# OpenGene/repaq

Hardware: AMD Instinct MI355X
Metric: raw FASTQ MB/s encode+decode (higher is better)
Workload: dtype u8; 1 GPU; configs[2]: synthetic NovaSeq PE150 two files (-i/-I), 2 x 4.01 GB FASTQ (fqgen profile 1, 11200000 pairs, seed 3, N 20 ppm), -k 1000, encode + decode; chunks_per_gpu=3360, parity=unchecked (checked with --full)

## Files before the change

repaq_amd/csrc/enc/chunk_flags_overlap.h:

```cpp
#pragma once
struct Layout {
    uint32_t off_readlens, off_n1lens, off_n2lens, off_stlens, off_lanes, off_tiles, off_x, off_y, off_n1, off_n2, off_st, off_seq, off_qual, off_ov, off_npos;
    uint32_t total, msize, seq_size, qual_size, npos_size, n1_size, n2_size, st_size, x_size, y_size, n_reads, flags;
};
__device__ __forceinline__ uint32_t name2_len_of(const Text& T, const ReadTab& R, uint32_t g) { return line_len(T, g, 0) - R.name2_off[g]; }

#define CF_ALL 0x3FFu
__global__ void k_chunk_flags_a(Text T, ReadTab R, ChunkTab C, const DevHeader* __restrict__ D, int is_pe, uint32_t* __restrict__ cbits, uint32_t* __restrict__ cfail) {
    __shared__ uint8_t s_names[4 * 65 * NAME_STRIDE];
    const uint32_t c = blockIdx.y, f = C.first[c], e = C.first[c + 1];
    const int l = lane_id(), w = wave_id(); const uint32_t wpb = blockDim.x >> 6;
    uint8_t* rows = s_names + (size_t)w * 65 * NAME_STRIDE;
    const bool can0 = is_pe && D->support_interleaved; const uint32_t dpos = D->name2_diff_pos, dch = D->name2_diff_char;
    const uint32_t nl0 = line_len(T, f, 0); const uint8_t* nm0g = line_ptr(T, f, 0);
    const uint32_t n1l0 = R.name1_len[f], n2o0 = R.name2_off[f], n2l0 = nl0 - n2o0, len0 = R.len[f], stl0 = line_len(T, f, 2);
    const uint8_t* st0 = line_ptr(T, f, 2); const uint8_t lane0 = R.lane[f]; const uint16_t tile0 = R.tile[f];
    { const uint32_t take = nl0 < NAME_CAP ? nl0 : NAME_CAP; for (uint32_t i = (uint32_t)l; i < take; i += 64) rows[64 * NAME_STRIDE + i] = nm0g[i]; }
    const uint8_t* nm0 = nl0 <= NAME_CAP ? rows + 64 * NAME_STRIDE : nm0g;
    uint32_t bits = CF_ALL, fail = 0xFFFFFFFFu;
    for (uint32_t gb = f + (blockIdx.x * wpb + (uint32_t)w) * 64u; gb < e; gb += gridDim.x * wpb * 64u) {
        const uint32_t g = gb + (uint32_t)l; const bool v = g < e;
        uint32_t nb = 0, nl = 0, stb = 0, stl = 0; int s = 0;
        if (v) { uint32_t r; read_loc(T, g, s, r); const uint32_t* p = t_lo(T, s) + 4 * (size_t)r; nb = p[0]; nl = p[1] - 1 - nb; stb = p[2]; stl = p[3] - 1 - stb; }
        wave_lds_sync();
// ... 314 lines not shown
__global__ void __launch_bounds__(256) k_chunk_prefix(Text T, ReadTab R, ChunkTab C, const DevHeader* __restrict__ D, const int16_t* __restrict__ ovraw,
        int8_t* __restrict__ ovb) {
    const uint32_t c = blockIdx.x, f = C.first[c], e = C.first[c + 1], tid = threadIdx.x;
    const bool enc = C.il[c] != 0 && (D->flags & H_PE_OVERLAP); const int shift = D->overlap_shift;
    const uint32_t fl = C.flags[c];
    const bool pieces = !(fl & C_NAME1_SAME) || ((D->flags & H_NAME2) && !(fl & C_NAME2_SAME)) || !(fl & C_STRAND_SAME);
    U4 carry; carry.a = carry.b = carry.c = carry.d = 0;
    for (uint32_t base = f; base < e; base += 1024u) {
        U4 v[4]; U4 acc; acc.a = acc.b = acc.c = acc.d = 0;
#pragma unroll
        for (int i = 0; i < 4; i++) {
            const uint32_t g = base + 4u * tid + (uint32_t)i; v[i].a = v[i].b = v[i].c = v[i].d = 0;
            if (g < e) {
                uint32_t st = R.len[g];
                if (enc && ((g - f) & 1u)) {
                    int ov = ovraw[g >> 1];
                    if (ov + shift > 127) ov = 0;
                    if (ov + shift < -127) ov = 0;
                    ovb[g >> 1] = (int8_t)(ov + shift); st -= (uint32_t)(ov < 0 ? -ov : ov); R.stored[g] = st;
                }
                if (pieces) { int s_; uint32_t r_; read_loc(T, g, s_, r_); const uint4 lo4 = *(const uint4*)(t_lo(T, s_) + 4 * (size_t)r_);
                        v[i].a = R.name1_len[g]; v[i].b = (lo4.y - 1u - lo4.x) - R.name2_off[g]; v[i].c = lo4.w - 1u - lo4.z; }
                v[i].d = st;
                acc = acc + v[i];
            }
        }
        U4 tot; U4 run = carry + block_excl_sum<U4>(acc, &tot);
#pragma unroll
        for (int i = 0; i < 4; i++) { const uint32_t g = base + 4u * tid + (uint32_t)i; if (g < e) { if (pieces) R.pv[g] = run; R.sd[g] = run.d; run = run + v[i]; } }
        carry = carry + tot;
    }
    if (tid == 0) { C.ptot[c] = carry; C.sbase[c] = C.qbase[c]; }
}
__global__ void k_chunk_ptot(ReadTab R, ChunkTab C, uint32_t n_chunks) {
    const uint32_t c = blockIdx.x * blockDim.x + threadIdx.x;
    if (c < n_chunks) C.ptot[c] = R.pv[C.first[c + 1]] - R.pv[C.first[c]];
}
```

repaq_amd/csrc/enc/gather_tiles.h:

```cpp
#pragma once
#define G2_CAP 23552u
#define G2_SE_OK 1
#define G2_CNT 256u
struct __attribute__((packed, aligned(1))) GU16g { uint32_t a, b, c, d; };
__device__ __forceinline__ void pack4_codes(uint32_t w, uint32_t& code, uint32_t& nb, uint32_t& bad) {
    const uint32_t idx = (w >> 1) & 0x03030303u;
    const uint32_t ok = eq_bytes_full(__builtin_amdgcn_perm(0u, 0x47544341u, idx), w);
    code = ((__builtin_amdgcn_perm(0u, 0x00020301u, idx) & ok) * 0x01041040u) >> 24;
    nb = 0; bad = 0;
    if (ok != 0xFFFFFFFFu) { const uint32_t isn = eq_bytes_full(w, 0x4E4E4E4Eu); nb = ((isn & 0x01010101u) * 0x01020408u) >> 24;
            bad = (((~ok & ~isn) & 0x01010101u) * 0x01020408u) >> 24; }
}
__device__ __forceinline__ void pack4_codes_rc(uint32_t w, uint32_t& code, uint32_t& nb) {
    const uint32_t u = w & 0xDFDFDFDFu, idx = (u >> 1) & 0x03030303u;
    const uint32_t ok = eq_bytes_full(__builtin_amdgcn_perm(0u, 0x47544341u, idx), u);
    code = ((__builtin_amdgcn_perm(0u, 0x03010002u, idx) & ok) * 0x01041040u) >> 24;
    nb = ((~ok & 0x01010101u) * 0x01020408u) >> 24;
}
__device__ __forceinline__ bool pack16_fast(const uint32_t (&w)[4], uint32_t& code) {
    uint32_t diff = 0; code = 0;
#pragma unroll
    for (int i = 0; i < 4; i++) {
        const uint32_t idx = (w[i] >> 1) & 0x03030303u;
        diff |= __builtin_amdgcn_perm(0u, 0x47544341u, idx) ^ w[i];
// ... 433 lines not shown
    const uint32_t nw = (pq[first[c + 1]] - pq[first[c]] + 31u) >> 5; const size_t w0 = (size_t)(qbase[c] >> 5);
    for (uint32_t v = 0; v < G2_PLANES; v++) if (!((dense_mask >> v) & 1u)) for (uint32_t i = threadIdx.x; i < nw; i += blockDim.x) planes[(size_t)v * pstride + w0 + i] = 0u;
}
__global__ void k_gather_redo_reset(const uint32_t* __restrict__ only, uint32_t* __restrict__ segm, int* __restrict__ segc, uint32_t n_seg,
                                    uint32_t* __restrict__ xplane, uint64_t pstride, const DevHeader* __restrict__ D, uint32_t nd, const uint32_t* __restrict__ pq, const uint32_t* __restrict__ first, const uint64_t* __restrict__ qbase) {
    const uint32_t c = blockIdx.x; if (!only[c]) return;
    const size_t k = (size_t)c * MAX_STREAMS * n_seg;
    for (uint32_t i = threadIdx.x; i < MAX_STREAMS * n_seg; i += blockDim.x) { segm[k + i] = 0u; segc[k + i] = -1; }
    if (xplane) { k_rare_zero_chunk(xplane, pstride, dense_mask_of(D, nd), pq, first, qbase, c);
            if (threadIdx.x == 0) xplane[(size_t)G2_PLANES * pstride + (size_t)c * (1u + G2_RARE_LIST)] = 0u; }
}
__global__ void k_rare_cleanup(uint32_t* __restrict__ rare, uint32_t* __restrict__ planes, uint64_t pstride, const DevHeader* __restrict__ D, uint32_t nd,
        const uint32_t* __restrict__ pq, const uint32_t* __restrict__ first, const uint64_t* __restrict__ qbase) {
    const uint32_t c = blockIdx.x; uint32_t* const rc = rare + (size_t)c * (1u + G2_RARE_LIST); const uint32_t n = rc[0]; if (!n) return;
    if (n <= G2_RARE_LIST) { const size_t w0 = (size_t)(qbase[c] >> 5); for (uint32_t i = threadIdx.x; i < n; i += blockDim.x) { const uint32_t e = rc[1u + i];
            planes[(size_t)(e >> 28) * pstride + w0 + (e & 0x0FFFFFFFu)] = 0u; } }
    else k_rare_zero_chunk(planes, pstride, dense_mask_of(D, nd), pq, first, qbase, c);
    __syncthreads();
    if (threadIdx.x == 0) rc[0] = 0u;
}
__device__ __forceinline__ uint32_t loose_codes(const uint32_t* __restrict__ lpk, uint32_t ld, uint32_t b) {
    const uint32_t d = ld + (b >> 4), sh = 2u * (b & 15u); const uint32_t lo = lpk[d];
    return sh ? (uint32_t)(((((unsigned long long)lpk[d + 1]) << 32) | lo) >> sh) : lo;
}
__device__ __forceinline__ uint32_t loose_nbits(const uint16_t* __restrict__ lnb, uint32_t ld, uint32_t b) {
    const uint32_t d = ld + (b >> 4), sh = b & 15u; const uint32_t lo = lnb[d];
    return (sh ? ((((uint32_t)lnb[d + 1]) << 16) | lo) >> sh : lo) & 0xFFFFu;
}
#define SP_OWN 4096u
#define SP_EXTRA 8u
#define SP_U 3
struct __attribute__((packed, aligned(4))) SpU8 { uint32_t a, b; };
struct __attribute__((packed, aligned(2))) SpU4 { uint32_t a; };
__global__ void __launch_bounds__(256) k_seqpack(const uint32_t* __restrict__ pq, const uint32_t* __restrict__ sd, const U4* __restrict__ ptot,
        const uint32_t* __restrict__ first, const uint32_t* __restrict__ ilv, const int8_t* __restrict__ ovb,
                                                 const DevHeader* __restrict__ D, const uint64_t* __restrict__ sbase, const uint32_t* __restrict__ lpk, const uint16_t* __restrict__ lnb, const uint8_t* __restrict__ rn,
                                                 uint32_t* __restrict__ spk, uint16_t* __restrict__ snm, uint32_t* __restrict__ ncount, uint32_t* __restrict__ nmap, uint32_t* __restrict__ segm, int* __restrict__ segc, uint32_t n_seg,
                                                 uint32_t rshift) {
    __shared__ uint32_t s_sd[256 + SP_EXTRA + 1], s_ld[256 + SP_EXTRA], s_sk[256 + SP_EXTRA]; __shared__ uint8_t s_own[SP_OWN];
    __shared__ uint8_t s_hn[256 + SP_EXTRA + 8];
    const uint32_t c = blockIdx.y, f = first[c], e = first[c + 1], tid = threadIdx.x;
    const uint32_t ps0 = sd[f], S = ptot[c].d;
    const bool il = ilv[c] != 0, enc = il && (D->flags & H_PE_OVERLAP); const int shift = D->overlap_shift;
    uint32_t* const ok = spk + (size_t)(sbase[c] >> 4); uint16_t* const on = snm + (size_t)(sbase[c] >> 4);
    const uint32_t nshift = nmap_shift(S); uint32_t* const nm = nmap + (size_t)c * NMAP_WORDS;
    const size_t nsi = ((size_t)c * MAX_STREAMS + NPOS_SLOT) * n_seg;
    uint32_t nsum = 0;
    auto skip_of = [&](uint32_t g) -> uint32_t {
        if (enc && ((g - f) & 1u)) { const int ov = (int)ovb[g >> 1] - shift; if (ov > 0) return (uint32_t)ov; }
        return 0u;
    };
    const uint32_t R = 1u << rshift;
    for (uint32_t r0 = f + blockIdx.x * R; r0 < e; r0 += gridDim.x * R) {
        const uint32_t nr = e - r0 < R ? e - r0 : R, nx = e - r0 < R + SP_EXTRA ? e - r0 : R + SP_EXTRA;
        for (uint32_t t = tid; t <= nx; t += blockDim.x) {
            const uint32_t g = r0 + t; s_sd[t] = g < e ? sd[g] - ps0 : S;
            if (t < nx) { s_ld[t] = (pq[g] >> 4) + g; s_sk[t] = skip_of(g); s_hn[t] = rn[g]; } else s_hn[t] = 0;
        }
        __syncthreads();
        const uint32_t kbase = (s_sd[0] + 15u) >> 4, kend = (s_sd[nr] + 15u) >> 4;
        if (tid < nr) { const uint32_t ka = (s_sd[tid] + 15u) >> 4, kb = (s_sd[tid + 1] + 15u) >> 4; for (uint32_t k = ka; k < kb; k++) s_own[k - kbase] = (uint8_t)tid; }
        __syncthreads();
        const uint32_t ndw = kend - kbase;
        for (uint32_t i0 = 0; i0 < ndw; i0 += blockDim.x * SP_U) {
            struct Dw { uint32_t k, need, t1, jj, sh, sh2, take2, n, n2; unsigned long long c, c2; } q[SP_U]; uint32_t nres[SP_U];
#pragma unroll
            for (int u = 0; u < SP_U; u++) nres[u] = 0;
#pragma unroll
            for (int u = 0; u < SP_U; u++) {
                Dw& x = q[u]; x.need = 0; x.take2 = 0; x.k = x.t1 = x.jj = x.sh = x.sh2 = x.n = x.n2 = 0; x.c = x.c2 = 0;
                const uint32_t i = i0 + (uint32_t)u * blockDim.x + tid;
                if (i < ndw) {
                    const uint32_t k = kbase + i, j = s_own[i];
                    const uint32_t B = 16u * k, si = B - s_sd[j], need = S - B < 16u ? S - B : 16u, av = s_sd[j + 1] - B, t1 = need < av ? need : av;
                    const uint32_t b0 = s_sk[j] + si, d = s_ld[j] + (b0 >> 4);
                    x.k = k; x.need = need; x.t1 = t1; x.sh = b0 & 15u; x.jj = j + 1u;
                    { const SpU8 v = *(const SpU8*)(lpk + d); x.c = (((unsigned long long)v.b) << 32) | v.a; x.n = s_hn[j] ? ((const SpU4*)(lnb + d))->a : 0u; }
                    if (t1 < need && j + 1u < nx) {
                        const uint32_t avail = s_sd[j + 2] - s_sd[j + 1]; x.jj = j + 2u;
                        if (avail) {
                            const uint32_t s2 = s_sk[j + 1], d2 = s_ld[j + 1] + (s2 >> 4); x.sh2 = s2 & 15u; x.take2 = avail < need - t1 ? avail : need - t1;
                            const SpU8 v = *(const SpU8*)(lpk + d2); x.c2 = (((unsigned long long)v.b) << 32) | v.a; x.n2 = s_hn[j + 1] ? ((const SpU4*)(lnb + d2))->a : 0u;
                        }
                    }
                }
            }
#pragma unroll
            for (int u = 0; u < SP_U; u++) {
                const Dw& x = q[u];
                if (!x.need) continue;
                const uint32_t k = x.k, B = 16u * k, need = x.need;
                unsigned long long acc = (uint32_t)(x.c >> (2u * x.sh)) & (x.t1 >= 16u ? 0xFFFFFFFFu : (1u << (2u * x.t1)) - 1u);
                uint32_t nacc = ((x.n >> x.sh) & 0xFFFFu) & ((1u << x.t1) - 1u);
                uint32_t filled = x.t1, jj = x.jj;
                if (x.take2) {
                    acc |= (unsigned long long)((uint32_t)(x.c2 >> (2u * x.sh2)) & (x.take2 >= 16u ? 0xFFFFFFFFu : (1u << (2u * x.take2)) - 1u)) << (2u * filled);
                    nacc |= (((x.n2 >> x.sh2) & 0xFFFFu) & ((1u << x.take2) - 1u)) << filled; filled += x.take2;
                }
                while (filled < need) {
                    uint32_t a, b, l2, s2;
                    if (jj < nx) { a = s_sd[jj]; b = s_sd[jj + 1]; l2 = s_ld[jj]; s2 = s_sk[jj]; }
                    else { const uint32_t gg = r0 + jj; a = sd[gg] - ps0; b = gg + 1u < e ? sd[gg + 1] - ps0 : S; l2 = (pq[gg] >> 4) + gg; s2 = skip_of(gg); }
                    const uint32_t avail = b - a;
                    if (avail) {
                        const uint32_t take = avail < need - filled ? avail : need - filled;
                        acc |= (unsigned long long)(loose_codes(lpk, l2, s2) & (take >= 16u ? 0xFFFFFFFFu : (1u << (2u * take)) - 1u)) << (2u * filled);
                        if (jj < nx ? s_hn[jj] : rn[r0 + jj]) nacc |= (loose_nbits(lnb, l2, s2) & ((1u << take) - 1u)) << filled;
                        filled += take;
                    }
                    jj++;
                }
                ok[k] = (uint32_t)acc; on[k] = (uint16_t)nacc; nres[u] = nacc;
            }
#pragma unroll
            for (int u = 0; u < SP_U; u++) {
                const uint32_t na = q[u].need ? nres[u] : 0u;
                const unsigned long long hn = __ballot(na != 0u);
                if (!hn) continue;
                const uint32_t B = 16u * q[u].k, sg = B / PC_SEG_POS, mb = (B >> 12) >> nshift, n = (uint32_t)__popc(na);
                const int lead = __ffsll((long long)hn) - 1;
                const uint32_t sg0 = (uint32_t)__shfl((int)sg, lead), mb0 = (uint32_t)__shfl((int)mb, lead);
                const bool mine = na != 0u && sg == sg0; const int last = na ? (int)(B + 31u - (uint32_t)__clz((int)na)) : -1;
                const uint32_t sum = wave_sum<uint32_t>(mine ? n : 0u); const int mx = wave_max<int>(mine ? last : -1);
                if (lane_id() == lead) { atomicAdd(&segm[nsi + sg0], sum); atomicMax(&segc[nsi + sg0], mx); atomicOr(&nm[mb0 >> 5], 1u << (mb0 & 31u)); }
                if (na != 0u && !mine) { atomicAdd(&segm[nsi + sg], n); atomicMax(&segc[nsi + sg], last); }
                if (na != 0u && mb != mb0) atomicOr(&nm[mb >> 5], 1u << (mb & 31u));
                nsum += n;
            }
        }
        __syncthreads();
    }
    nsum = wave_sum(nsum);
    if (lane_id() == 0 && nsum) atomicAdd(&ncount[c], nsum);
}
// ... 47 lines not shown
```

repaq_amd/csrc/rfq_api.hip:

```cpp
#include "rfq_ctx.h"
#include <cstring>
#include <algorithm>
#include <new>
#include <cstdlib>
#include <string>
#include <cerrno>

extern "C" const char* rfq_version(void) {
#ifdef RFQ_SIMT_EMULATION
    return "rfq_hip 0.1.0 simt-emulation (test build, not a product path)";
#else
    return "rfq_hip 0.1.0 gfx950";
#endif
}

static bool opt_num(const std::string& v, long long lo, long long hi, long long* out) {
    if (v.empty()) return false;
    errno = 0; char* end = nullptr; const long long x = strtoll(v.c_str(), &end, 10);
    if (errno || !end || *end || end == v.c_str() || x < lo || x > hi) return false;
    *out = x; return true;
}
extern "C" int rfq_set_option(rfq_ctx* c, const char* name, const char* value) {
    if (!c || !name) return RFQ_E_ARG;
    const std::string n = name, v = value ? value : ""; const bool set = !v.empty(); const RfqOpts d; long long num = 0;
#define RFQ_OPT_NUM(LO, HI, WHAT) if (set && !opt_num(v, LO, HI, &num)) return rfq_fail(c, RFQ_E_ARG, "%s is " WHAT " (got \"%s\")", name, v.c_str());
    if (n == "RFQ_GATHER") { if (set && v != "old" && v != "tile") return rfq_fail(c, RFQ_E_ARG, "RFQ_GATHER is old or tile"); c->opt.gather_old = v == "old"; }
    else if (n == "RFQ_QUAL") { if (set && v != "bytes" && v != "masks") return rfq_fail(c, RFQ_E_ARG, "RFQ_QUAL is bytes or masks"); c->opt.qual_bytes = v == "bytes"; }
    else if (n == "RFQ_CODER") { if (set && v != "list" && v != "mask") return rfq_fail(c, RFQ_E_ARG, "RFQ_CODER is list or mask");
            c->opt.coder = v == "list" ? 1 : (v == "mask" ? 2 : 0); }
    else if (n == "RFQ_INDEX") { if (set && v != "2pass" && v != "1pass") return rfq_fail(c, RFQ_E_ARG, "RFQ_INDEX is 2pass or 1pass"); c->opt.index_2pass = v == "2pass"; }
    else if (n == "RFQ_IDX_TILES") { if (set && v != "4" && v != "8" && v != "16") return rfq_fail(c, RFQ_E_ARG, "RFQ_IDX_TILES is 4, 8 or 16");
            c->opt.idx_tiles = set ? atoi(v.c_str()) : d.idx_tiles; }
    else if (n == "RFQ_STREAMS") { if (set && v != "1" && v != "2") return rfq_fail(c, RFQ_E_ARG, "RFQ_STREAMS is 1 or 2"); c->opt.one_stream = v == "1"; }
    else if (n == "RFQ_SLICE_BYTES") { RFQ_OPT_NUM(1024, 0xFFFFFFF0ll - 16, "a number of bytes in 1024 .. 2^32 - 32") c->opt.slice_bytes = set ? (size_t)num : 0; }
    else if (n == "RFQ_SLICE_BASES") { RFQ_OPT_NUM(1, 0xFFFFFFF0ll, "a number of bases in 1 .. 2^32 - 16") c->opt.slice_bases = set ? (uint64_t)num : 0; }
    else if (n == "RFQ_WALK") { if (set && v != "exact" && v != "guess") return rfq_fail(c, RFQ_E_ARG, "RFQ_WALK is guess or exact"); c->opt.walk_exact = v == "exact"; }
    else if (n == "RFQ_GW_SHIFT") { RFQ_OPT_NUM(4, 30, "4 .. 30") c->opt.gw_shift = set ? (int)num : d.gw_shift; }
    else if (n == "RFQ_MATERIALISE") { if (set && v != "0" && v != "1") return rfq_fail(c, RFQ_E_ARG, "RFQ_MATERIALISE is 0 or 1"); c->opt.materialise = v == "1"; }
    else if (n == "RFQ_TRACE") { if (set && v != "0" && v != "1") return rfq_fail(c, RFQ_E_ARG, "RFQ_TRACE is 0 or 1"); c->opt.trace = v == "1"; }
    else if (n == "RFQ_G2_PAD") { RFQ_OPT_NUM(0, 150000, "0 .. 150000 bytes of LDS") c->opt.g2_pad = set ? (uint32_t)num : 0u; }
    else if (n == "RFQ_SP_PAD") { RFQ_OPT_NUM(0, 150000, "0 .. 150000 bytes of LDS") c->opt.sp_pad = set ? (uint32_t)num : d.sp_pad; }
    else if (n == "RFQ_POS_SEG") { if (set && v != "1024" && v != "2048") return rfq_fail(c, RFQ_E_ARG, "RFQ_POS_SEG is 1024 or 2048"); c->opt.pos_seg = set ? atoi(v.c_str()) : 0; }
    else if (n == "RFQ_SPEC") { if (set && v != "0" && v != "1") return rfq_fail(c, RFQ_E_ARG, "RFQ_SPEC is 0 or 1"); c->opt.no_spec = v == "0"; }
    else return rfq_fail(c, RFQ_E_ARG, "unknown option %s", name);
#undef RFQ_OPT_NUM
    return RFQ_OK;
}
static const char* const RFQ_OPTION_NAMES[] = { "RFQ_GATHER", "RFQ_QUAL", "RFQ_CODER", "RFQ_INDEX", "RFQ_IDX_TILES", "RFQ_STREAMS", "RFQ_SLICE_BYTES", "RFQ_SLICE_BASES", "RFQ_WALK", "RFQ_GW_SHIFT", "RFQ_MATERIALISE", "RFQ_TRACE", "RFQ_G2_PAD", "RFQ_SP_PAD", "RFQ_POS_SEG", "RFQ_SPEC" };
extern "C" const char* rfq_option_name(int i) { return (i >= 0 && i < (int)(sizeof RFQ_OPTION_NAMES / sizeof RFQ_OPTION_NAMES[0])) ? RFQ_OPTION_NAMES[i] : nullptr; }
extern "C" int rfq_get_option(const rfq_ctx* c, const char* name, char* out, size_t cap) {
    if (!c || !name || !out || !cap) return RFQ_E_ARG;
    const std::string n = name; const RfqOpts& o = c->opt; const RfqOpts d; std::string v;
    if (n == "RFQ_GATHER") v = o.gather_old ? "old" : "";
    else if (n == "RFQ_QUAL") v = o.qual_bytes ? "bytes" : "";
    else if (n == "RFQ_CODER") v = o.coder == 1 ? "list" : (o.coder == 2 ? "mask" : "");
    else if (n == "RFQ_INDEX") v = o.index_2pass ? "2pass" : "";
    else if (n == "RFQ_IDX_TILES") v = o.idx_tiles != d.idx_tiles ? std::to_string(o.idx_tiles) : "";
    else if (n == "RFQ_STREAMS") v = o.one_stream ? "1" : "";
    else if (n == "RFQ_SLICE_BYTES") v = o.slice_bytes ? std::to_string(o.slice_bytes) : "";
    else if (n == "RFQ_SLICE_BASES") v = o.slice_bases ? std::to_string(o.slice_bases) : "";
    else if (n == "RFQ_WALK") v = o.walk_exact ? "exact" : "";
    else if (n == "RFQ_GW_SHIFT") v = o.gw_shift != d.gw_shift ? std::to_string(o.gw_shift) : "";
    else if (n == "RFQ_MATERIALISE") v = o.materialise ? "1" : "";
    else if (n == "RFQ_TRACE") v = o.trace ? "1" : "";
    else if (n == "RFQ_G2_PAD") v = o.g2_pad ? std::to_string(o.g2_pad) : "";
    else if (n == "RFQ_SP_PAD") v = o.sp_pad != d.sp_pad ? std::to_string(o.sp_pad) : "";
    else if (n == "RFQ_POS_SEG") v = o.pos_seg ? std::to_string(o.pos_seg) : "";
    else if (n == "RFQ_SPEC") v = o.no_spec ? "0" : "";
    else return RFQ_E_ARG;
    if (v.size() + 1 > cap) return RFQ_E_NOSPACE;
    memcpy(out, v.c_str(), v.size() + 1);
    return RFQ_OK;
}

extern "C" int rfq_create(rfq_ctx** out, int device_id) {
    if (!out) return RFQ_E_ARG;
    *out = nullptr;
    int n = 0;
    if (hipGetDeviceCount(&n) != hipSuccess || n <= 0) return RFQ_E_NO_DEVICE;
    if (device_id < 0 || device_id >= n) return RFQ_E_NO_DEVICE;
    if (hipSetDevice(device_id) != hipSuccess) return RFQ_E_NO_DEVICE;
    rfq_ctx* c = new (std::nothrow) rfq_ctx();
    if (!c) return RFQ_E_HIP;
    c->device = device_id;
    { int cu = 0; if (hipDeviceGetAttribute(&cu, hipDeviceAttributeMultiprocessorCount, device_id) == hipSuccess && cu > 0) c->n_cu = (uint32_t)cu; }
    if (hipStreamCreate(&c->stream) != hipSuccess) { delete c; return RFQ_E_NO_DEVICE; }
// ... 217 lines not shown
```

repaq_amd/csrc/rfq_ctx.h:

```cpp
#pragma once
#include "rfq_common.h"
#include "../../include/rfq_hip.h"
#include <cstring>
#include <string>
#include <vector>
#include <cstdio>
#include <cstdarg>
#include <algorithm>

struct DBuf {
    void* p = nullptr; size_t cap = 0;
    hipError_t ensure(size_t n) {
        if (n <= cap) return hipSuccess;
        if (p) { (void)hipFree(p); p = nullptr; cap = 0; }
        size_t want = n + n / 4 + 4096;
        hipError_t e = hipMalloc(&p, want);
        if (e != hipSuccess) { p = nullptr; return e; }
        cap = want; return hipSuccess;
    }
    hipError_t ensure_keep(size_t n, size_t keep, hipStream_t s) {
        if (n <= cap) return hipSuccess;
        void* q = nullptr; const size_t want = n + n / 2 + 4096;
        hipError_t e = hipMalloc(&q, want);
        if (e != hipSuccess) return e;
// ... 17 lines not shown
    void end(hipStream_t s) { (void)hipEventRecord(stages[used].b, s); used++; }
    void collect() {
        ms.assign(used, 0.f); names.assign(used, nullptr);
        for (size_t i = 0; i < used; i++) { (void)hipEventElapsedTime(&ms[i], stages[i].a, stages[i].b); names[i] = stages[i].name; }
    }
    void destroy() { for (auto& s : stages) { (void)hipEventDestroy(s.a); (void)hipEventDestroy(s.b); } stages.clear(); }
};
struct StageSums {
    std::vector<std::pair<const char*, float>> v;
    void add(const StageTimer& t) {
        for (size_t i = 0; i < t.names.size(); i++) {
            auto q = std::find_if(v.begin(), v.end(), [&](const std::pair<const char*, float>& e) { return e.first == t.names[i]; });
            if (q == v.end()) v.emplace_back(t.names[i], t.ms[i]); else q->second += t.ms[i];
        }
    }
    void publish(StageTimer& t) const { t.names.clear(); t.ms.clear(); for (auto& q : v) { t.names.push_back(q.first); t.ms.push_back(q.second); } }
};

static inline uint32_t grid_x_for(uint32_t n_chunks, uint32_t tiles_per_chunk, uint32_t slots) {
    uint32_t best = 1; double best_eff = 0.0;
    if (!n_chunks || !slots) return 1;
    for (uint32_t k = 6; k <= 12; k++) {
        uint32_t bx = (uint32_t)(((uint64_t)k * slots + n_chunks / 2) / n_chunks);
        bx = std::max<uint32_t>(1u, std::min<uint32_t>(std::max<uint32_t>(bx, 1u), tiles_per_chunk));
        const double rounds = (double)bx * n_chunks / slots, full = (double)(uint64_t)(rounds + 0.999999), eff = full > 0 ? rounds / full : 0.0;
        if (eff > best_eff + 1e-3) { best = bx; best_eff = eff; }
    }
    return best;
}
struct RfqOpts {
    int  coder = 0;
    bool qual_bytes = false;
    bool gather_old = false;
    bool index_2pass = false;
    int  idx_tiles = 0;
    bool one_stream = false;
    size_t slice_bytes = 0;
    uint64_t slice_bases = 0;
    bool walk_exact = false;
    int  gw_shift = 16;
    bool materialise = false;
    bool trace = false;
    uint32_t g2_pad = 0;
    uint32_t sp_pad = 0;
    bool no_spec = false;
    int  pos_seg = 0;
};
struct rfq_ctx {
    RfqOpts opt;
    bool e3_pieces_failed = false;
    int device = 0; uint32_t n_cu = 256;
    hipStream_t stream = nullptr; bool own_stream = false;
    hipStream_t aux = nullptr; hipEvent_t ev_fork = nullptr, ev_join = nullptr, ev_mid = nullptr;
    hipStream_t aux2 = nullptr; hipEvent_t ev_f = nullptr;
    hipEvent_t ev_ovl = nullptr;
    hipStream_t copy = nullptr; hipEvent_t copy_ev[64] = {}; uint64_t copy_next = 0, copy_done = 0;
    bool aux_ready() {
        if (aux) return true;
        if (hipStreamCreateWithFlags(&aux, hipStreamNonBlocking) != hipSuccess) { aux = nullptr; return false; }
        if (hipEventCreateWithFlags(&ev_fork, hipEventDisableTiming) != hipSuccess || hipEventCreateWithFlags(&ev_join, hipEventDisableTiming) != hipSuccess ||
            hipEventCreateWithFlags(&ev_mid, hipEventDisableTiming) != hipSuccess) return false;
        if (hipStreamCreateWithFlags(&aux2, hipStreamNonBlocking) != hipSuccess) { aux2 = nullptr; return false; }
        if (hipEventCreateWithFlags(&ev_f, hipEventDisableTiming) != hipSuccess) return false;
        if (hipEventCreateWithFlags(&ev_ovl, hipEventDisableTiming) != hipSuccess) return false;
        return true;
    }
// ... 114 lines not shown
```

repaq_amd/csrc/rfq_encode.hip:

```cpp
#include "rfq_ctx.h"
#include "rfq_encode_kernels.h"
#include <algorithm>
#include <cstring>
#include <cstdlib>
#include <cstddef>

enum EncBuf {
    B_BITMAP0 = 0, B_BITMAP1, B_BLK0, B_BLK1, B_LO0, B_LO1, B_SCANTMP,
    B_LEN, B_N1LEN, B_N2OFF, B_X, B_Y, B_TILE, B_LANE, B_OK, B_CHUNK, B_STORED, B_EQ2, B_PQ, B_PV, B_PVIN,
    B_ULEN, B_P, B_MINMAX, B_FIRST, B_CFLAGS, B_IL, B_HIST, B_NCOUNT, B_SCAP, B_SOFF, B_SSIZE, B_XSIZE, B_YSIZE, B_QBASE, B_SBASE,
    B_IMGSIZE, B_IMGOFF, B_CTOTAL, B_CBASE, B_LAYOUT, B_HSTATS, B_OVB, B_OVRAW, B_QCAT, B_SCAT, B_SCRATCH, B_XS, B_YS, B_SEGB, B_SEGC,
    B_NORM0, B_NORM1, B_OT0, B_OT1, B_ONX0, B_ONX1, B_TBITS, B_SBITS, B_NKEEP, B_NTERM, B_NMAP, B_ADJ, B_PINFO, B_SEGM, B_LPK, B_LNB, B_SPK, B_SNM, B_RFLAG, B_SCANTMP2, B_CTOTALN, B_CBASEN, B_SCRATCHN, B_PTOT, B_QPLANE, B_SEGD, B_SEGS, B_SD, B_RN, B_ENC_END
};

static_assert(B_ENC_END <= 80, "encode buffers must stay below the decode buffer indices of rfq_ctx::b");

static int fetch_bytes(rfq_ctx* ctx, const uint8_t* d, size_t n, std::string& out) {
    out.resize(n);
    if (n) HIPCHK(ctx, hipMemcpy(&out[0], d, n, hipMemcpyDeviceToHost));
    return RFQ_OK;
}
static int fetch_line(rfq_ctx* ctx, const Text& T, uint32_t g, int k, std::string& out) {
    int s = 0; uint32_t r = g; if (T.paired == 1) { s = (int)(g & 1u); r = g >> 1; }
    uint32_t lo2[2];
// ... 550 lines not shown
        }
        const uint32_t dyn = dyn_of(M.nd) + ctx->opt.g2_pad; (void)dyn;
        for (int phase = 1; phase <= (is_pe ? 2 : 1); phase++) {
            const uint32_t* only = phase == 2 ? (const uint32_t*)redo : (const uint32_t*)nullptr;
            if (phase == 2) hipLaunchKernelGGL(k_gather_redo_reset, dim3(n_chunks), dim3(64), 0, S, only, B[B_SEGM].as<uint32_t>(), B[B_SEGC].as<int>(), n_seg,
                                               masks ? M.planes : (uint32_t*)nullptr, M.pstride, (const DevHeader*)D, M.nd, (const uint32_t*)R.pq, (const uint32_t*)C.first, (const uint64_t*)C.qbase);
            if (masks) hipLaunchKernelGGL(k_mask_bounds, dim3(n_chunks), dim3(64), 0, S, (const uint32_t*)R.pq, (const uint32_t*)C.first, (const uint64_t*)C.qbase,
                    M.planes, M.pstride, (const DevHeader*)D, M.nd, bx, only);
#define RFQ_G2_ARGS T, R, (const uint32_t*)C.first, (const uint64_t*)C.qbase, (const DevHeader*)D, B[B_QCAT].as<uint8_t>(), B[B_LPK].as<uint32_t>(), B[B_LNB].as<uint16_t>(), B[B_RFLAG].as<uint8_t>(), \
                    B[B_RN].as<uint8_t>(), B[B_SEGM].as<uint32_t>(), B[B_SEGC].as<int>(), n_seg, kshift, cbits, cfail, only, text4, M
            if (masks && !is_pe && G2_SE_OK) hipLaunchKernelGGL((k_gather2<true, 0>), dim3(bx, n_chunks), dim3(256), dyn, S, RFQ_G2_ARGS);
            else if (masks && a->paired == RFQ_PE_TWO_FILES && G2_SE_OK) hipLaunchKernelGGL((k_gather2<true, 1>), dim3(bx, n_chunks), dim3(256), dyn, S, RFQ_G2_ARGS);
            else if (masks) hipLaunchKernelGGL(k_gather2<true>, dim3(bx, n_chunks), dim3(256), dyn, S, RFQ_G2_ARGS);
            else hipLaunchKernelGGL(k_gather2<false>, dim3(bx, n_chunks), dim3(256), dyn, S, RFQ_G2_ARGS);
#undef RFQ_G2_ARGS
            if (phase == 1) hipLaunchKernelGGL(k_chunk_flags_b, dim3(n_chunks), dim3(64), 0, S, R, C, (const DevHeader*)D, is_pe ? 1 : 0, (const uint32_t*)cbits,
                    (const uint32_t*)cfail, redo);
        }
        HIPCHK(ctx, B[B_SCRATCH].ensure(std::max<size_t>(B[B_SCRATCH].cap, (size_t)(masks ? total_bases / 8 : total_bases + total_bases / 4) + nc * 4096 + 256)));
        HIPCHK(ctx, B[B_SCRATCHN].ensure(std::max<size_t>(B[B_SCRATCHN].cap, (size_t)(total_bases / 64) + nc * 1024 + 256)));
        hipLaunchKernelGGL(k_stream_plan, dim3(n_chunks), dim3(64), 0, S, R, C, (const DevHeader*)D, ctot, ctot_n, n_chunks, (const uint32_t*)B[B_SEGM].as<uint32_t>(),
                n_seg, 1);
        scan_exclusive<uint64_t>(S, ctot, cbase, n_chunks, B[B_SCANTMP].as<uint64_t>(), 1);
        hipLaunchKernelGGL(k_enc_totals, dim3(1), dim3(64), 0, S, C, (const uint64_t*)cbase, n_chunks, 0, dst, (uint64_t)B[B_SCRATCH].cap);
        aux_chain = ctx->aux_ready() && !ctx->opt.one_stream; hipStream_t A = aux_chain ? ctx->aux : S;
        if (aux_chain) { HIPCHK(ctx, hipEventRecord(ctx->ev_fork, S)); HIPCHK(ctx, hipStreamWaitEvent(A, ctx->ev_fork, 0)); ovl_guard.armed = true; }
        if (is_pe) {
            const OvLoose Z = { (const uint32_t*)R.pq, (const uint32_t*)B[B_LPK].as<uint32_t>(), (const uint16_t*)B[B_LNB].as<uint16_t>(), (const uint8_t*)B[B_RFLAG].as<uint8_t>() };
            const uint32_t ob = std::min<uint32_t>((np + 255) / 256, 65535u * 16u);
            if (hs.max_len <= 160u) hipLaunchKernelGGL((k_overlap<true, 160u>), dim3(ob), dim3(256), 0, A, T, Z, B[B_OVRAW].as<int16_t>(), np);
            else hipLaunchKernelGGL(k_overlap<true>, dim3(ob), dim3(256), 0, A, T, Z, B[B_OVRAW].as<int16_t>(), np);
        }
        if (aux_chain) { HIPCHK(ctx, hipEventRecord(ctx->ev_ovl, A)); coder_waits = true; }
        hipLaunchKernelGGL(k_chunk_prefix, dim3(n_chunks), dim3(256), 0, A, T, R, C, (const DevHeader*)D, (const int16_t*)B[B_OVRAW].as<int16_t>(), ovb);
        {
            const uint32_t max_len = max_rec / 2u;
            uint32_t rshift = 8; while (rshift && ((uint64_t)(max_len / 16u + 1u) << rshift) > SP_OWN) rshift--;
            uint32_t sx = grid_x_for(n_chunks, (max_reads >> rshift) + 1u, 8u * ctx->n_cu);
            hipLaunchKernelGGL(k_seqpack, dim3(sx, n_chunks), dim3(256), aux_chain ? ctx->opt.sp_pad : 0u, A, (const uint32_t*)R.pq, (const uint32_t*)R.sd, (const U4*)C.ptot,
                    (const uint32_t*)C.first, (const uint32_t*)C.il, (const int8_t*)ovb, (const DevHeader*)D,
                               (const uint64_t*)C.sbase, (const uint32_t*)B[B_LPK].as<uint32_t>(), (const uint16_t*)B[B_LNB].as<uint16_t>(), (const uint8_t*)B[B_RN].as<uint8_t>(), B[B_SPK].as<uint32_t>(), B[B_SNM].as<uint16_t>(),
                               C.ncount, C.nmap, B[B_SEGM].as<uint32_t>(), B[B_SEGC].as<int>(), n_seg, rshift);
        }
        uint64_t* tmp2 = B[B_SCANTMP2].as<uint64_t>() + (nr / SCAN_TILE + 2) * 2;
        hipLaunchKernelGGL(k_stream_plan, dim3(n_chunks), dim3(64), 0, A, R, C, (const DevHeader*)D, ctot, ctot_n, n_chunks, (const uint32_t*)B[B_SEGM].as<uint32_t>(),
                n_seg, 2);
        scan_exclusive<uint64_t>(A, ctot_n, cbase_n, n_chunks, tmp2, 1);
        hipLaunchKernelGGL(k_chunk_layout, dim3((n_chunks + 63) / 64), dim3(64), 0, A, T, R, C, (const DevHeader*)D, L, n_chunks, 0, dst);
        scan_exclusive<uint64_t>(A, C.img_size, C.img_off, n_chunks, tmp2, 1);
        hipLaunchKernelGGL(k_enc_totals, dim3(1), dim3(64), 0, A, C, (const uint64_t*)cbase_n, n_chunks, 2, dst, (uint64_t)B[B_SCRATCHN].cap);
        KCHK(ctx, "k_gather2");
    } else {
        HIPCHK(ctx, B[B_SCAT].ensure(catbytes));
        const uint32_t bx = grid_x_for(n_chunks, (max_reads + GT_READS - 1) / GT_READS, 5u * ctx->n_cu);
        hipLaunchKernelGGL(k_gather, dim3(bx, n_chunks), dim3(256), 0, S, T, R, C, (const int8_t*)ovb, (const DevHeader*)D, B[B_QCAT].as<uint8_t>(),
                B[B_SCAT].as<uint8_t>(), B[B_SEGM].as<uint32_t>(), B[B_SEGC].as<int>(), n_seg);
        const uint32_t px = grid_x_for(n_chunks, (hs.max_chunk_bases / 16u + 255u) / 256u + 1u, 8u * ctx->n_cu);
        hipLaunchKernelGGL(k_packbytes, dim3(px, n_chunks), dim3(256), 0, S, (const U4*)R.pv, (const uint32_t*)C.first, (const uint64_t*)C.sbase,
                (const uint8_t*)B[B_SCAT].as<uint8_t>(),
                           B[B_SPK].as<uint32_t>(), B[B_SNM].as<uint16_t>());
        hipLaunchKernelGGL(k_stream_plan, dim3(n_chunks), dim3(64), 0, S, R, C, (const DevHeader*)D, ctot, ctot_n, n_chunks, (const uint32_t*)B[B_SEGM].as<uint32_t>(),
                n_seg, 3);
        scan_exclusive<uint64_t>(S, ctot, cbase, n_chunks, B[B_SCANTMP].as<uint64_t>(), 1);
        scan_exclusive<uint64_t>(S, ctot_n, cbase_n, n_chunks, B[B_SCANTMP].as<uint64_t>(), 1);
        hipLaunchKernelGGL(k_chunk_layout, dim3((n_chunks + 63) / 64), dim3(64), 0, S, T, R, C, (const DevHeader*)D, L, n_chunks, 0, dst);
        scan_exclusive<uint64_t>(S, C.img_size, C.img_off, n_chunks, B[B_SCANTMP].as<uint64_t>(), 1);
        hipLaunchKernelGGL(k_enc_totals, dim3(1), dim3(64), 0, S, C, (const uint64_t*)cbase, n_chunks, 0, dst, ~0ull);
        hipLaunchKernelGGL(k_enc_totals, dim3(1), dim3(64), 0, S, C, (const uint64_t*)cbase_n, n_chunks, 2, dst, ~0ull);
        KCHK(ctx, "k_gather");
    }
    if (!fast) {
        HIPCHK(ctx, ctx->fetch(&hs, dst, sizeof hs, S));
        if (make_header) HIPCHK(ctx, ctx->fetch(&ctx->h_hdr, D, sizeof(DevHeader), S));
        HIPCHK(ctx, ctx->fetch_sync(S));
    }
// ... 127 lines not shown
```

Baseline: 1.097 million MB/s.

## Fuse chunk prefix scan into seqpack, recomputing stored offsets on the fly

Removes the separate k_chunk_prefix launch. k_seqpack now derives per-read stored-sequence offsets from the pq prefix minus a running block scan of clamped overlap values, and writes ovb itself. Block 0 of each chunk computes name and strand piece prefixes only when the chunk flags need them, and otherwise writes ptot and sbase directly. This saves a kernel launch plus a full pass writing and re-reading sd and pv. In exchange every seqpack block re-reduces the overlap values preceding its own reads, which adds redundant work, and block 0 can serialise on the pieces prefix. The old chain is still available through RFQ_PACK=chain.

Result: slower. 1.074 million MB/s (-2.1%).

```diff
diff --git a/repaq_amd/csrc/enc/chunk_flags_overlap.h b/repaq_amd/csrc/enc/chunk_flags_overlap.h
--- a/repaq_amd/csrc/enc/chunk_flags_overlap.h
+++ b/repaq_amd/csrc/enc/chunk_flags_overlap.h
@@ -370,6 +370,25 @@
     }
     if (tid == 0) { C.ptot[c] = carry; C.sbase[c] = C.qbase[c]; }
 }
+__device__ __forceinline__ int ov_clamped(int ov, int shift) { if (ov + shift > 127) ov = 0; if (ov + shift < -127) ov = 0; return ov; }
+__device__ __forceinline__ void chunk_pieces_prefix(const Text& T, const ReadTab& R, const ChunkTab& C, const DevHeader* __restrict__ D, const int16_t* __restrict__ ovraw, uint32_t c) {
+    const uint32_t f = C.first[c], e = C.first[c + 1], tid = threadIdx.x;
+    const bool enc = C.il[c] != 0 && (D->flags & H_PE_OVERLAP); const int shift = D->overlap_shift;
+    U4 carry; carry.a = carry.b = carry.c = carry.d = 0;
+    for (uint32_t base = f; base < e; base += blockDim.x) {
+        const uint32_t g = base + tid; U4 v; v.a = v.b = v.c = v.d = 0;
+        if (g < e) {
+            uint32_t st = R.len[g];
+            if (enc && ((g - f) & 1u)) { const int ov = ov_clamped(ovraw[g >> 1], shift); st -= (uint32_t)(ov < 0 ? -ov : ov); }
+            int s_; uint32_t r_; read_loc(T, g, s_, r_); const uint4 lo4 = *(const uint4*)(t_lo(T, s_) + 4 * (size_t)r_);
+            v.a = R.name1_len[g]; v.b = (lo4.y - 1u - lo4.x) - R.name2_off[g]; v.c = lo4.w - 1u - lo4.z; v.d = st;
+        }
+        U4 tot; const U4 run = carry + block_excl_sum<U4>(v, &tot);
+        if (g < e) R.pv[g] = run;
+        carry = carry + tot;
+    }
+    if (tid == 0) { C.ptot[c] = carry; C.sbase[c] = C.qbase[c]; }
+}
 __global__ void k_chunk_ptot(ReadTab R, ChunkTab C, uint32_t n_chunks) {
     const uint32_t c = blockIdx.x * blockDim.x + threadIdx.x;
     if (c < n_chunks) C.ptot[c] = R.pv[C.first[c + 1]] - R.pv[C.first[c]];
diff --git a/repaq_amd/csrc/enc/gather_tiles.h b/repaq_amd/csrc/enc/gather_tiles.h
--- a/repaq_amd/csrc/enc/gather_tiles.h
+++ b/repaq_amd/csrc/enc/gather_tiles.h
@@ -489,32 +489,67 @@
 #define SP_U 3
 struct __attribute__((packed, aligned(4))) SpU8 { uint32_t a, b; };
 struct __attribute__((packed, aligned(2))) SpU4 { uint32_t a; };
-__global__ void __launch_bounds__(256) k_seqpack(const uint32_t* __restrict__ pq, const uint32_t* __restrict__ sd, const U4* __restrict__ ptot,
+struct SpFused { Text T; ReadTab R; ChunkTab C; const int16_t* ovraw; int8_t* ovb; };
+template <bool FUSED> __global__ void __launch_bounds__(256) k_seqpack(const uint32_t* __restrict__ pq, const uint32_t* __restrict__ sd, const U4* __restrict__ ptot,
         const uint32_t* __restrict__ first, const uint32_t* __restrict__ ilv, const int8_t* __restrict__ ovb,
                                                  const DevHeader* __restrict__ D, const uint64_t* __restrict__ sbase, const uint32_t* __restrict__ lpk, const uint16_t* __restrict__ lnb, const uint8_t* __restrict__ rn,
                                                  uint32_t* __restrict__ spk, uint16_t* __restrict__ snm, uint32_t* __restrict__ ncount, uint32_t* __restrict__ nmap, uint32_t* __restrict__ segm, int* __restrict__ segc, uint32_t n_seg,
-                                                 uint32_t rshift) {
+                                                 uint32_t rshift, SpFused Z) {
     __shared__ uint32_t s_sd[256 + SP_EXTRA + 1], s_ld[256 + SP_EXTRA], s_sk[256 + SP_EXTRA]; __shared__ uint8_t s_own[SP_OWN];
     __shared__ uint8_t s_hn[256 + SP_EXTRA + 8];
     const uint32_t c = blockIdx.y, f = first[c], e = first[c + 1], tid = threadIdx.x;
-    const uint32_t ps0 = sd[f], S = ptot[c].d;
     const bool il = ilv[c] != 0, enc = il && (D->flags & H_PE_OVERLAP); const int shift = D->overlap_shift;
-    uint32_t* const ok = spk + (size_t)(sbase[c] >> 4); uint16_t* const on = snm + (size_t)(sbase[c] >> 4);
+    const uint32_t pq0 = pq[f];
+    auto ov_of = [&](uint32_t g) -> int { return (enc && ((g - f) & 1u)) ? ov_clamped(Z.ovraw[g >> 1], shift) : 0; };
+    auto aov_of = [&](uint32_t g) -> uint32_t { const int ov = ov_of(g); return (uint32_t)(ov < 0 ? -ov : ov); };
+    uint32_t ps0 = 0, S = 0, acar = 0, apos = f;
+    if (FUSED) {
+        uint32_t a = 0, atot = 0;
+        if (enc) for (uint32_t g = f + 1u + 2u * tid; g < e; g += 2u * blockDim.x) a += aov_of(g);
+        block_excl_sum<uint32_t>(a, &atot);
+        S = (pq[e] - pq0) - atot;
+        if (blockIdx.x == 0) {
+            const uint32_t fl = Z.C.flags[c];
+            if (!(fl & C_NAME1_SAME) || ((D->flags & H_NAME2) && !(fl & C_NAME2_SAME)) || !(fl & C_STRAND_SAME)) chunk_pieces_prefix(Z.T, Z.R, Z.C, D, Z.ovraw, c);
+            else if (tid == 0) { U4 t; t.a = t.b = t.c = 0; t.d = S; Z.C.ptot[c] = t; Z.C.sbase[c] = Z.C.qbase[c]; }
+        }
+    } else { ps0 = sd[f]; S = ptot[c].d; }
+    const uint64_t sb = FUSED ? Z.C.qbase[c] : sbase[c];
+    uint32_t* const ok = spk + (size_t)(sb >> 4); uint16_t* const on = snm + (size_t)(sb >> 4);
     const uint32_t nshift = nmap_shift(S); uint32_t* const nm = nmap + (size_t)c * NMAP_WORDS;
     const size_t nsi = ((size_t)c * MAX_STREAMS + NPOS_SLOT) * n_seg;
     uint32_t nsum = 0;
     auto skip_of = [&](uint32_t g) -> uint32_t {
+        if (FUSED) { const int ov = ov_of(g); return ov > 0 ? (uint32_t)ov : 0u; }
         if (enc && ((g - f) & 1u)) { const int ov = (int)ovb[g >> 1] - shift; if (ov > 0) return (uint32_t)ov; }
         return 0u;
     };
     const uint32_t R = 1u << rshift;
     for (uint32_t r0 = f + blockIdx.x * R; r0 < e; r0 += gridDim.x * R) {
         const uint32_t nr = e - r0 < R ? e - r0 : R, nx = e - r0 < R + SP_EXTRA ? e - r0 : R + SP_EXTRA;
+        if (FUSED) {
+            if (apos < r0) {
+                uint32_t a = 0, t = 0;
+                if (enc) for (uint32_t g = apos + tid; g < r0; g += blockDim.x) a += aov_of(g);
+                block_excl_sum<uint32_t>(a, &t); acar += t;
+            }
+            const uint32_t g = r0 + tid; const int ov = tid < nx ? ov_of(g) : 0; uint32_t tot = 0;
+            const uint32_t x = block_excl_sum<uint32_t>((uint32_t)(ov < 0 ? -ov : ov), &tot);
+            if (tid <= nx) s_sd[tid] = g < e ? (pq[g] - pq0) - (acar + x) : S;
+            if (tid < nx) { s_ld[tid] = (pq[g] >> 4) + g; s_sk[tid] = ov > 0 ? (uint32_t)ov : 0u; s_hn[tid] = rn[g]; } else if (tid == nx) s_hn[tid] = 0;
+            if (tid < nr && enc && ((g - f) & 1u)) Z.ovb[g >> 1] = (int8_t)(ov + shift);
+            for (uint32_t t = blockDim.x + tid; t <= nx; t += blockDim.x) {
+                const uint32_t g2 = r0 + t; uint32_t ex = 0; for (uint32_t u = blockDim.x; u < t; u++) ex += aov_of(r0 + u);
+                s_sd[t] = g2 < e ? (pq[g2] - pq0) - (acar + tot + ex) : S;
+                if (t < nx) { s_ld[t] = (pq[g2] >> 4) + g2; s_sk[t] = skip_of(g2); s_hn[t] = rn[g2]; } else s_hn[t] = 0;
+            }
+        } else
         for (uint32_t t = tid; t <= nx; t += blockDim.x) {
             const uint32_t g = r0 + t; s_sd[t] = g < e ? sd[g] - ps0 : S;
             if (t < nx) { s_ld[t] = (pq[g] >> 4) + g; s_sk[t] = skip_of(g); s_hn[t] = rn[g]; } else s_hn[t] = 0;
         }
         __syncthreads();
+        if (FUSED && r0 + nr < e) { acar = (pq[r0 + nr] - pq0) - s_sd[nr]; apos = r0 + nr; }
         const uint32_t kbase = (s_sd[0] + 15u) >> 4, kend = (s_sd[nr] + 15u) >> 4;
         if (tid < nr) { const uint32_t ka = (s_sd[tid] + 15u) >> 4, kb = (s_sd[tid + 1] + 15u) >> 4; for (uint32_t k = ka; k < kb; k++) s_own[k - kbase] = (uint8_t)tid; }
         __syncthreads();
@@ -549,7 +584,7 @@
                 const uint32_t k = x.k, B = 16u * k, need = x.need;
                 unsigned long long acc = (uint32_t)(x.c >> (2u * x.sh)) & (x.t1 >= 16u ? 0xFFFFFFFFu : (1u << (2u * x.t1)) - 1u);
                 uint32_t nacc = ((x.n >> x.sh) & 0xFFFFu) & ((1u << x.t1) - 1u);
-                uint32_t filled = x.t1, jj = x.jj;
+                uint32_t filled = x.t1, jj = x.jj, tail = 0;
                 if (x.take2) {
                     acc |= (unsigned long long)((uint32_t)(x.c2 >> (2u * x.sh2)) & (x.take2 >= 16u ? 0xFFFFFFFFu : (1u << (2u * x.take2)) - 1u)) << (2u * filled);
                     nacc |= (((x.n2 >> x.sh2) & 0xFFFFu) & ((1u << x.take2) - 1u)) << filled; filled += x.take2;
@@ -557,6 +592,8 @@
                 while (filled < need) {
                     uint32_t a, b, l2, s2;
                     if (jj < nx) { a = s_sd[jj]; b = s_sd[jj + 1]; l2 = s_ld[jj]; s2 = s_sk[jj]; }
+                    else if (FUSED) { const uint32_t gg = r0 + jj; a = jj == nx ? s_sd[nx] : tail; b = gg + 1u < e ? a + (pq[gg + 1] - pq[gg]) - aov_of(gg) : S; tail = b;
+                            l2 = (pq[gg] >> 4) + gg; s2 = skip_of(gg); }
                     else { const uint32_t gg = r0 + jj; a = sd[gg] - ps0; b = gg + 1u < e ? sd[gg + 1] - ps0 : S; l2 = (pq[gg] >> 4) + gg; s2 = skip_of(gg); }
                     const uint32_t avail = b - a;
                     if (avail) {
diff --git a/repaq_amd/csrc/rfq_api.hip b/repaq_amd/csrc/rfq_api.hip
--- a/repaq_amd/csrc/rfq_api.hip
+++ b/repaq_amd/csrc/rfq_api.hip
@@ -25,6 +25,7 @@
     const std::string n = name, v = value ? value : ""; const bool set = !v.empty(); const RfqOpts d; long long num = 0;
 #define RFQ_OPT_NUM(LO, HI, WHAT) if (set && !opt_num(v, LO, HI, &num)) return rfq_fail(c, RFQ_E_ARG, "%s is " WHAT " (got \"%s\")", name, v.c_str());
     if (n == "RFQ_GATHER") { if (set && v != "old" && v != "tile") return rfq_fail(c, RFQ_E_ARG, "RFQ_GATHER is old or tile"); c->opt.gather_old = v == "old"; }
+    else if (n == "RFQ_PACK") { if (set && v != "chain" && v != "fused") return rfq_fail(c, RFQ_E_ARG, "RFQ_PACK is chain or fused"); c->opt.pack_chain = v == "chain"; }
     else if (n == "RFQ_QUAL") { if (set && v != "bytes" && v != "masks") return rfq_fail(c, RFQ_E_ARG, "RFQ_QUAL is bytes or masks"); c->opt.qual_bytes = v == "bytes"; }
     else if (n == "RFQ_CODER") { if (set && v != "list" && v != "mask") return rfq_fail(c, RFQ_E_ARG, "RFQ_CODER is list or mask");
             c->opt.coder = v == "list" ? 1 : (v == "mask" ? 2 : 0); }
@@ -46,12 +47,13 @@
 #undef RFQ_OPT_NUM
     return RFQ_OK;
 }
-static const char* const RFQ_OPTION_NAMES[] = { "RFQ_GATHER", "RFQ_QUAL", "RFQ_CODER", "RFQ_INDEX", "RFQ_IDX_TILES", "RFQ_STREAMS", "RFQ_SLICE_BYTES", "RFQ_SLICE_BASES", "RFQ_WALK", "RFQ_GW_SHIFT", "RFQ_MATERIALISE", "RFQ_TRACE", "RFQ_G2_PAD", "RFQ_SP_PAD", "RFQ_POS_SEG", "RFQ_SPEC" };
+static const char* const RFQ_OPTION_NAMES[] = { "RFQ_GATHER", "RFQ_QUAL", "RFQ_CODER", "RFQ_INDEX", "RFQ_IDX_TILES", "RFQ_STREAMS", "RFQ_SLICE_BYTES", "RFQ_SLICE_BASES", "RFQ_WALK", "RFQ_GW_SHIFT", "RFQ_MATERIALISE", "RFQ_TRACE", "RFQ_G2_PAD", "RFQ_SP_PAD", "RFQ_POS_SEG", "RFQ_SPEC", "RFQ_PACK" };
 extern "C" const char* rfq_option_name(int i) { return (i >= 0 && i < (int)(sizeof RFQ_OPTION_NAMES / sizeof RFQ_OPTION_NAMES[0])) ? RFQ_OPTION_NAMES[i] : nullptr; }
 extern "C" int rfq_get_option(const rfq_ctx* c, const char* name, char* out, size_t cap) {
     if (!c || !name || !out || !cap) return RFQ_E_ARG;
     const std::string n = name; const RfqOpts& o = c->opt; const RfqOpts d; std::string v;
     if (n == "RFQ_GATHER") v = o.gather_old ? "old" : "";
+    else if (n == "RFQ_PACK") v = o.pack_chain ? "chain" : "";
     else if (n == "RFQ_QUAL") v = o.qual_bytes ? "bytes" : "";
     else if (n == "RFQ_CODER") v = o.coder == 1 ? "list" : (o.coder == 2 ? "mask" : "");
     else if (n == "RFQ_INDEX") v = o.index_2pass ? "2pass" : "";
diff --git a/repaq_amd/csrc/rfq_ctx.h b/repaq_amd/csrc/rfq_ctx.h
--- a/repaq_amd/csrc/rfq_ctx.h
+++ b/repaq_amd/csrc/rfq_ctx.h
@@ -73,6 +73,7 @@
     int  coder = 0;
     bool qual_bytes = false;
     bool gather_old = false;
+    bool pack_chain = false;
     bool index_2pass = false;
     int  idx_tiles = 0;
     bool one_stream = false;
diff --git a/repaq_amd/csrc/rfq_encode.hip b/repaq_amd/csrc/rfq_encode.hip
--- a/repaq_amd/csrc/rfq_encode.hip
+++ b/repaq_amd/csrc/rfq_encode.hip
@@ -606,15 +606,21 @@
             else hipLaunchKernelGGL(k_overlap<true>, dim3(ob), dim3(256), 0, A, T, Z, B[B_OVRAW].as<int16_t>(), np);
         }
         if (aux_chain) { HIPCHK(ctx, hipEventRecord(ctx->ev_ovl, A)); coder_waits = true; }
-        hipLaunchKernelGGL(k_chunk_prefix, dim3(n_chunks), dim3(256), 0, A, T, R, C, (const DevHeader*)D, (const int16_t*)B[B_OVRAW].as<int16_t>(), ovb);
+        const bool pack_fused = !ctx->opt.pack_chain;
+        if (!pack_fused) hipLaunchKernelGGL(k_chunk_prefix, dim3(n_chunks), dim3(256), 0, A, T, R, C, (const DevHeader*)D, (const int16_t*)B[B_OVRAW].as<int16_t>(), ovb);
         {
             const uint32_t max_len = max_rec / 2u;
             uint32_t rshift = 8; while (rshift && ((uint64_t)(max_len / 16u + 1u) << rshift) > SP_OWN) rshift--;
             uint32_t sx = grid_x_for(n_chunks, (max_reads >> rshift) + 1u, 8u * ctx->n_cu);
-            hipLaunchKernelGGL(k_seqpack, dim3(sx, n_chunks), dim3(256), aux_chain ? ctx->opt.sp_pad : 0u, A, (const uint32_t*)R.pq, (const uint32_t*)R.sd, (const U4*)C.ptot,
-                    (const uint32_t*)C.first, (const uint32_t*)C.il, (const int8_t*)ovb, (const DevHeader*)D,
-                               (const uint64_t*)C.sbase, (const uint32_t*)B[B_LPK].as<uint32_t>(), (const uint16_t*)B[B_LNB].as<uint16_t>(), (const uint8_t*)B[B_RN].as<uint8_t>(), B[B_SPK].as<uint32_t>(), B[B_SNM].as<uint16_t>(),
-                               C.ncount, C.nmap, B[B_SEGM].as<uint32_t>(), B[B_SEGC].as<int>(), n_seg, rshift);
+            const SpFused ZF = { T, R, C, (const int16_t*)B[B_OVRAW].as<int16_t>(), ovb };
+#define RFQ_SP_ARGS (const uint32_t*)C.first, (const uint32_t*)C.il, pack_fused ? (const int8_t*)nullptr : (const int8_t*)ovb, (const DevHeader*)D, \
+                               (const uint64_t*)C.sbase, (const uint32_t*)B[B_LPK].as<uint32_t>(), (const uint16_t*)B[B_LNB].as<uint16_t>(), (const uint8_t*)B[B_RN].as<uint8_t>(), B[B_SPK].as<uint32_t>(), B[B_SNM].as<uint16_t>(), \
+                               C.ncount, C.nmap, B[B_SEGM].as<uint32_t>(), B[B_SEGC].as<int>(), n_seg, rshift, ZF
+            if (pack_fused) hipLaunchKernelGGL(k_seqpack<true>, dim3(sx, n_chunks), dim3(256), aux_chain ? ctx->opt.sp_pad : 0u, A, (const uint32_t*)R.pq, (const uint32_t*)nullptr,
+                    (const U4*)nullptr, RFQ_SP_ARGS);
+            else hipLaunchKernelGGL(k_seqpack<false>, dim3(sx, n_chunks), dim3(256), aux_chain ? ctx->opt.sp_pad : 0u, A, (const uint32_t*)R.pq, (const uint32_t*)R.sd, (const U4*)C.ptot,
+                    RFQ_SP_ARGS);
+#undef RFQ_SP_ARGS
         }
         uint64_t* tmp2 = B[B_SCANTMP2].as<uint64_t>() + (nr / SCAN_TILE + 2) * 2;
         hipLaunchKernelGGL(k_stream_plan, dim3(n_chunks), dim3(64), 0, A, R, C, (const DevHeader*)D, ctot, ctot_n, n_chunks, (const uint32_t*)B[B_SEGM].as<uint32_t>(),
```
